# Boese0601/RC-MVSNet

Measured on AMD Instinct MI355X. Metric: ref-scenes/sec (DTU 3-view 512x640, D=48/32/8), higher is better.
Workload: dtype f32; 1 GPU; BASELINE configs[1]: CascadeMVSNet_eval.forward, DTU-shaped 3 views 512x640, D=(48,32,8), batch 1 per GPU, fp32, random-init seeded weights; views=3, height=512, width=640, parallelism=scene-per-gpu x1, ranks=1, procs_per_gpu=1, rccl_ranks=0

## Files before the change

rc_mvsnet_amd/casmvsnet.py:

```python
import os

FP16_PAIR_DEFAULT = True
ONE_BY_ONE_MFMA = os.environ.get("RCMVS_1X1_MFMA", "1") != "0"
HEAD_PAIR = os.environ.get("RCMVS_HEAD_PAIR", "1") != "0"
CONV11_PROB = int(os.environ.get("RCMVS_CONV11_PROB", "1"))
CONV_TILE = os.environ.get("RCMVS_CONV_TILE", "1") != "0"
CONV_STEM = os.environ.get("RCMVS_CONV_STEM", "1") != "0"
CONV_PAIR = os.environ.get("RCMVS_CONV_PAIR", "1") != "0"
DEEP_PAIR = os.environ.get("RCMVS_DEEP_PAIR", "1") != "0"

import torch
import torch.nn as nn
import torch.nn.functional as F

from . import ops
from ._lib import RcmvsError


def _nhwc(x):
    x = x.contiguous().float()
    return ops.rgb_to_nhwc4(x) if x.shape[1] == 3 else ops.to_channels_last(x)


def _param(mod, name):
    p = mod._parameters.get(name)
    return p if p is not None else getattr(mod, name)


def _packed_of(module, make):
    w = module.conv.weight
    key = (w.data_ptr(), w._version, str(w.device))
    c = module.__dict__.get("_rcmvs_pack")
    if c is None or c[0] != key:
        c = module.__dict__["_rcmvs_pack"] = (key, make(w.detach()))
    return c[1]


def _affine_of(m):
    if getattr(m, "gn", None) is not None:
        raise RcmvsError(f"{type(m).__name__}: GroupNorm blocks are not provided (the reference builds every block with norm='batch_norm')")
    if m.bn is not None:
        return _bn_fold(m.bn)
    b = m.conv.bias
    if b is None:
        return None, None
    return torch.ones_like(b, dtype=torch.float32), b.detach().float().contiguous()


def _same2(v, n):
    return tuple(v) == (n, n)


def _conv2d_block_cl(m, t):
    conv = m.conv
    K = conv.kernel_size[0]
    st = conv.stride[0]
    if (not _same2(conv.kernel_size, K) or K not in (1, 3, 5) or not _same2(conv.padding, K // 2) or not _same2(conv.stride, st)
            or st not in (1, 2) or not _same2(conv.dilation, 1) or conv.groups != 1 or conv.padding_mode != "zeros"):
# ... 618 lines not shown
        depth = None
        bounds = None
        need_fill = False
        pair = getattr(self, "fp16_pair", None)
        if pair is None:
            pair = FP16_PAIR_DEFAULT if os.environ.get("RCMVS_FP16_PAIR") is None else os.environ["RCMVS_FP16_PAIR"] == "1"
        if pair and B == 1:
            bounds = getattr(self, "_pair_bounds", None)
            if getattr(self, "_is_replica", False):
                bounds = torch.zeros(self.num_stage, CostRegNet.BOUND_ROWS, ops.ABSMAX_FLOATS, device=imgs.device, dtype=torch.float32)
            elif bounds is None or bounds.device != imgs.device:
                bounds = self._pair_bounds = torch.zeros(self.num_stage, CostRegNet.BOUND_ROWS, ops.ABSMAX_FLOATS, device=imgs.device, dtype=torch.float32)
            else:
                need_fill = True
        if homographies is None:
            if self.num_stage <= 4:
                rots, transs = ops.compose_homography_stages([proj_matrices["stage{}".format(k + 1)].contiguous().float() for k in range(self.num_stage)],
                                                             zero=bounds if need_fill else None)
                need_fill = False
            else:
                rt = [ops.compose_homography(proj_matrices["stage{}".format(k + 1)].contiguous().float()) for k in range(self.num_stage)]
                rots, transs = [r for r, _ in rt], [t for _, t in rt]
        if need_fill:
            bounds.zero_()
        for s in range(self.num_stage):
            key = "stage{}".format(s + 1)
            scale = int(self.stage_infos[key]["scale"])
            D = self.ndepths[s]
            bound_kept = False
            if feats_cl is not None:
                fk, bound_kept = feats_cl[key](bounds[s][0] if bounds is not None else None)
                h, w, C = fk.shape[1:]
                f_cl = fk.view(B, V, h, w, C)
            else:
                C, h, w = features[key].shape[1:]
                f_cl = ops.to_channels_last(features[key].contiguous()).view(B, V, h, w, C)
            if homographies is not None:
                rot, trans = homographies[key]
            else:
                rot, trans = rots[s], transs[s]
            planes = ops.hypothesis_planes(depth, depth_values, (H, W), scale, D, self.depth_interals_ratio[s])
            var = ops.warp_variance(f_cl, rot, trans, planes, D, uniform_planes=depth is None)
            cr = self._cr(s)
            vmax = None
            if bounds is not None:
                vmax = bounds[s]
                if not bound_kept:
                    ops.absmax(f_cl, square=True, out=vmax[0])
            plan = cr.hip_plan()
            if vmax is not None and HEAD_PAIR and (CONV11_PROB == 2 or (CONV11_PROB == 1 and D == 8)):
                depth, conf = cr.features_cl(var, vmax, plan, logits=True, planes=planes)
            else:
                x8 = cr.features_cl(var, vmax, plan)
                depth, conf = ops.depth_head(x8, plan["prob"], planes, x_absmax=vmax[CostRegNet.BOUND_ROWS - 1] if vmax is not None and HEAD_PAIR else None)
            out = {"depth": depth, "photometric_confidence": conf}
            if self.TRAIN_VARIANT:
                small_cl = ops.resize_rgb_cl(imgs.reshape(B * V, 3, H, W).contiguous(), (h, w)).view(B, V, h, w, 3)
                out["volume_feature_no_ref"] = ops.warp_noref(f_cl, small_cl, rot, trans, planes, D, square_first=True)
            outputs[key] = out
            outputs.update(out)
        return outputs

    def _forward_train_hip(self, imgs, proj_matrices, depth_values):
        from . import train_ops
        B, V, _, H, W = imgs.shape
        imgs = imgs.float()
        depth_values = depth_values.contiguous().float()
        fv = self.feature.forward_train_cl(imgs.transpose(0, 1).reshape(V * B, 3, H, W), segments=V)
        features = [{k: f[v * B:(v + 1) * B] for k, f in fv.items()} for v in range(V)]
        outputs = {}
        depth = None
        for s in range(self.num_stage):
            key = "stage{}".format(s + 1)
            scale = int(self.stage_infos[key]["scale"])
            D = self.ndepths[s]
            f_cl = torch.stack([f[key] for f in features], dim=1).contiguous()
            h, w = f_cl.shape[2:4]
            with torch.no_grad():
                rot, trans = ops.compose_homography(proj_matrices[key].contiguous().float())
                prev = depth.detach() if depth is not None else None
                planes = ops.hypothesis_planes(prev, depth_values, (H, W), scale, D, self.depth_interals_ratio[s])
                small_cl = None
                if self.TRAIN_VARIANT:
                    small_cl = ops.resize_rgb_cl(imgs.reshape(B * V, 3, H, W).contiguous(), (h, w)).view(B, V, h, w, 3)
            res = ops.WarpVarianceFn.apply(f_cl, rot, trans, planes, D, small_cl)
            var, noref = res if self.TRAIN_VARIANT else (res, None)
            cr = self._cr(s)
            x8 = cr.features_cl_train(var)
            prev_live = depth
            depth, conf = train_ops.ProbDepthHeadFn.apply(x8, cr.prob.weight, planes)
            if prev_live is not None and self.grad_method != "detach":
                up = F.interpolate(prev_live.unsqueeze(1), [H, W], mode="bilinear", align_corners=False)
                base = F.interpolate(up, [h, w], mode="bilinear", align_corners=False).squeeze(1)
                depth = depth + (base - base.detach())
            out = {"depth": depth, "photometric_confidence": conf}
            if self.TRAIN_VARIANT:
                out["volume_feature_no_ref"] = noref
            outputs[key] = out
            outputs.update(out)
        return outputs

    def _run(self, imgs, proj_matrices, depth_values):
        if _hip_inference(self, imgs, depth_values):
            return self._forward_hip(imgs, proj_matrices, depth_values)
        if _hip_training(self, imgs, depth_values):
            return self._forward_train_hip(imgs, proj_matrices, depth_values)
        _unsupported(self, imgs, depth_values)
# ... 16 lines not shown
```

rc_mvsnet_amd/csrc/depth_head.hip:

```cpp
#include "common.h"

namespace rcmvs {

int conv3d_lds_launch(const float* x, const float* wp, const float* scale, const float* shift, const float* res, float* y,
                      int B, int D, int H, int W, int Ci, int Co, int relu, hipStream_t st, int lds_cfg);
bool prob_head_fused_supported(int D, int H, int W);
bool prob_pair_supported(int D, int H, int W);
int prob_pair_launch(const float* x, const float* wimg, const float* xmax, float* y, const float* planes, float* depth, float* conf,
                     int B, int D, int H, int W, bool fuse, int zc_force, hipStream_t st);
long long prob_pair_blob_offset();
int prob_head_fused_launch(const float* x, const float* wp, const float* planes, float* depth, float* conf, float* prob,
                           int B, int D, int H, int W, hipStream_t st);

template <int LP, bool KEEP = true>
__global__ __launch_bounds__(256) void softmax_regress_kernel(float* __restrict__ prob, const float* __restrict__ planes,
                                                               float* __restrict__ depth, float* __restrict__ conf, int D, long long hw) {
    constexpr int MAXK = 16;
    const int b = blockIdx.y;
    const int j = threadIdx.x % LP;
    const long long p = ((long long)blockIdx.x * blockDim.x + threadIdx.x) / LP;
    const bool live = p < hw;
    float* col = prob + (long long)b * D * hw + (live ? p : 0);
    float v[MAXK];
    float mx = -INFINITY;
#pragma unroll
    for (int i = 0; i < MAXK; ++i) {
        const int k = j + i * LP;
        v[i] = (k < D) ? col[(long long)k * hw] : -INFINITY;
        mx = fmaxf(mx, v[i]);
    }
#pragma unroll
    for (int m = 1; m < LP; m <<= 1) mx = fmaxf(mx, __shfl_xor(mx, m));
    float sum = 0.0f;
#pragma unroll
    for (int i = 0; i < MAXK; ++i) {
        v[i] = (j + i * LP < D) ? expf(v[i] - mx) : 0.0f;
        sum += v[i];
    }
#pragma unroll
    for (int m = 1; m < LP; m <<= 1) sum += __shfl_xor(sum, m);
    const float2 pl = reinterpret_cast<const float2*>(planes)[(long long)b * hw + (live ? p : 0)];
    float dsum = 0.0f, isum = 0.0f;
#pragma unroll
    for (int i = 0; i < MAXK; ++i) {
        const int k = j + i * LP;
        v[i] = v[i] / sum;
        if (k < D) {
            if (KEEP && live) col[(long long)k * hw] = v[i];
            dsum = fmaf(v[i], fmaf((float)k, pl.y, pl.x), dsum);
            isum = fmaf(v[i], (float)k, isum);
        }
    }
#pragma unroll
    for (int m = 1; m < LP; m <<= 1) { dsum += __shfl_xor(dsum, m); isum += __shfl_xor(isum, m); }
    int idx = (int)isum;
    idx = idx < 0 ? 0 : (idx > D - 1 ? D - 1 : idx);
    float c = 0.0f;
#pragma unroll
    for (int i = 0; i < MAXK; ++i) {
        const int k = j + i * LP;
        if (k < D && k >= idx - 1 && k <= idx + 2) c += v[i];
    }
#pragma unroll
    for (int m = 1; m < LP; m <<= 1) c += __shfl_xor(c, m);
    if (live && j == 0) {
        depth[(long long)b * hw + p] = dsum;
        conf[(long long)b * hw + p] = c;
    }
}

}

using namespace rcmvs;

static int depth_head_fwd(const float* x, const float* xmax, const float* w_prob, const float* planes, float* depth, float* conf, float* prob,
                          int B, int D, int h, int w, int impl, void* stream) {
    RCMVS_REQUIRE(x && w_prob && planes && depth && conf, "depth_head_fwd: null pointer");
    RCMVS_REQUIRE(B > 0 && D > 0 && h > 0 && w > 0, "depth_head_fwd: bad sizes");
    RCMVS_REQUIRE(D <= 64, "depth_head_fwd: at most 64 depth hypotheses per stage (got %d)", D);
    hipStream_t st = as_stream(stream);
    const int zc_force = (impl >> 8) & 0xff;
    const bool pair = xmax && !(impl & 4) && prob_pair_supported(D, h, w);
    int rc;
    if (pair && D == 8 && !(impl & 1))
        return prob_pair_launch(x, w_prob + prob_pair_blob_offset(), xmax, prob, planes, depth, conf, B, D, h, w, true, 0, st);
    if (!pair && !(impl & 1) && prob_head_fused_supported(D, h, w)) return prob_head_fused_launch(x, w_prob, planes, depth, conf, prob, B, D, h, w, st);
    RCMVS_REQUIRE(prob, "depth_head_fwd: prob is required for D = %d (it doubles as the logit scratch; only the D = 8 form runs without)", D);
    if (pair) rc = prob_pair_launch(x, w_prob + prob_pair_blob_offset(), xmax, prob, nullptr, nullptr, nullptr, B, D, h, w, false, zc_force, st);
    else rc = conv3d_lds_launch(x, w_prob, nullptr, nullptr, nullptr, prob, B, D, h, w, 8, 1, 0, st, ((impl & 2) ? 16 : 0) | (zc_force << 8));
    if (rc) return rc;
    const long long hw = (long long)h * w;
    const bool keep = !(impl & 8);
#define RCMVS_SOFTMAX(LP) do { if (keep) hipLaunchKernelGGL((softmax_regress_kernel<LP, true>), dim3((unsigned)cdiv(hw * LP, 256), B), dim3(256), 0, st, prob, planes, depth, conf, D, hw); \
                               else hipLaunchKernelGGL((softmax_regress_kernel<LP, false>), dim3((unsigned)cdiv(hw * LP, 256), B), dim3(256), 0, st, prob, planes, depth, conf, D, hw); } while (0)
    if (D <= 16) RCMVS_SOFTMAX(1);
    else if (D <= 32) RCMVS_SOFTMAX(2);
    else RCMVS_SOFTMAX(4);
#undef RCMVS_SOFTMAX
    return launch_status("depth_head_fwd");
}

extern "C" int rcmvs_softmax_head_fwd(float* prob, const float* planes, float* depth, float* conf, int B, int D, int h, int w, int keep, void* stream) {
    RCMVS_REQUIRE(prob && planes && depth && conf, "softmax_head_fwd: null pointer");
    RCMVS_REQUIRE(B > 0 && D > 0 && h > 0 && w > 0, "softmax_head_fwd: bad sizes");
    RCMVS_REQUIRE(D <= 64, "softmax_head_fwd: at most 64 depth hypotheses per stage (got %d)", D);
    hipStream_t st = as_stream(stream);
    const long long hw = (long long)h * w;
#define RCMVS_SOFTMAX(LP) do { if (keep) hipLaunchKernelGGL((softmax_regress_kernel<LP, true>), dim3((unsigned)cdiv(hw * LP, 256), B), dim3(256), 0, st, prob, planes, depth, conf, D, hw); \
                               else hipLaunchKernelGGL((softmax_regress_kernel<LP, false>), dim3((unsigned)cdiv(hw * LP, 256), B), dim3(256), 0, st, prob, planes, depth, conf, D, hw); } while (0)
    if (D <= 16) RCMVS_SOFTMAX(1);
    else if (D <= 32) RCMVS_SOFTMAX(2);
    else RCMVS_SOFTMAX(4);
#undef RCMVS_SOFTMAX
    return launch_status("softmax_head_fwd");
}

extern "C" int rcmvs_depth_head_fwd(const float* x, const float* w_prob, const float* planes, float* depth, float* conf, float* prob,
                                    int B, int D, int h, int w, void* stream) {
    return depth_head_fwd(x, nullptr, w_prob, planes, depth, conf, prob, B, D, h, w, 0, stream);
}
extern "C" int rcmvs_depth_head_scaled_fwd(const float* x, const float* x_absmax, const float* w_prob, const float* planes, float* depth, float* conf,
                                           float* prob, int B, int D, int h, int w, int impl, void* stream) {
    return depth_head_fwd(x, x_absmax, w_prob, planes, depth, conf, prob, B, D, h, w, impl, stream);
}
```

rc_mvsnet_amd/csrc/prob_pair.hip:

```cpp
#include "common.h"
#include "x3_pieces.h"
#include <type_traits>

namespace rcmvs {

constexpr int PP_TH = 8, PP_TW = 32, PP_HH = PP_TH + 2, PP_HW = PP_TW + 2;
constexpr int PP_PIECE = PP_HH * PP_HW * 16;
constexpr int PP_BUF = 2 * PP_PIECE;
constexpr int PP_NLD = (PP_HH * PP_HW * 2 + 255) / 256;
constexpr int PP_NJ = 3, PP_STEP = 14;

long long prob_pair_weight_floats() { return 4 + 3 * 2 * 64 * 4; }

__global__ void prob_pair_pack_kernel(const float* __restrict__ w, unsigned short* __restrict__ img, const float* __restrict__ wsc) {
    const int t = blockIdx.x * blockDim.x + threadIdx.x;
    if (t >= 3 * 64 * 8) return;
    const int c = t & 7, lane = (t >> 3) & 63, r = t >> 9;
    const int m = lane & 15, kh = lane >> 4, g = m >> 2, kw = m & 3;
    float v = 0.0f;
    if (g < 3 && kw < 3 && kh < 3) {
        const int kd = (g + r) % 3;
        v = w[c * 27 + (kd * 3 + kh) * 3 + kw];
    }
    const float sw = wsc[0];
    if (t == 0) { float* hdr = reinterpret_cast<float*>(img); hdr[0] = sw; hdr[1] = wsc[1]; hdr[2] = 0.0f; hdr[3] = 0.0f; }
    const float vs = v * sw;
    const _Float16 h = (_Float16)vs;
    const _Float16 l = (_Float16)(vs - (float)h);
    const int base = 8 + ((r * 2) * 64 + lane) * 8 + c;
    img[base] = __builtin_bit_cast(unsigned short, h);
    img[base + 64 * 8] = __builtin_bit_cast(unsigned short, l);
}

int prob_pair_pack(const float* w, float* img, const float* wsc, hipStream_t st) {
    hipLaunchKernelGGL(prob_pair_pack_kernel, dim3(6), dim3(256), 0, st, w, reinterpret_cast<unsigned short*>(img), wsc);
    return launch_status("prob_pair_pack");
}

template <int FUSE_D>
__global__ __launch_bounds__(256, 4) void prob_pair_kernel(
    const float* __restrict__ x, const x3_u32x4* __restrict__ wimg, const float* __restrict__ xmax, float* __restrict__ y,
    int D, int H, int W, int tiles_w, int tiles_h, int zchunk,
    const float* __restrict__ planes, float* __restrict__ depth, float* __restrict__ conf) {
    constexpr int LGB = FUSE_D > 0 ? FUSE_D * 256 * 4 : 0;
    __shared__ __attribute__((aligned(16))) x3_byte smem[2 * PP_BUF + LGB + 16];
    constexpr int OOB = 0x7ffffff0;
    const int tid = threadIdx.x, lane = tid & 63;
    const int wave = __builtin_amdgcn_readfirstlane(tid >> 6);
    const int n = lane & 15, kq = lane >> 4;
    const int b = blockIdx.z, zc = blockIdx.y;
    const unsigned t2 = xcd_remap(blockIdx.x, gridDim.x);
    const int tw = t2 % tiles_w, th = t2 / tiles_w;
    const int h0 = th * PP_TH, w0 = tw * PP_TW, z0 = zc * zchunk;
    const int z1 = min(D, z0 + zchunk);
    const int nplanes = z1 - z0 + 2;
    const int plane_bytes = H * W * 32;
    const float xmax_lane = xmax[lane * 16];
    const float whdr = reinterpret_cast<const float*>(wimg)[1];
    __amdgpu_buffer_rsrc_t xrs = __builtin_amdgcn_make_buffer_rsrc(const_cast<float*>(x + (long long)b * D * H * W * 8), (short)0, D * plane_bytes, 0x00020000);
    __amdgpu_buffer_rsrc_t yrs = __builtin_amdgcn_make_buffer_rsrc(y ? y + (long long)b * D * H * W : nullptr, (short)0, y ? D * H * W * 4 : 0, 0x00020000);
    int goff[PP_NLD], ls[PP_NLD];
#pragma unroll
    for (int i = 0; i < PP_NLD; ++i) {
        const int e = tid + i * 256;
        const int v = e >> 1, c4 = e & 1;
        const int hh = v / PP_HW, hw_ = v - hh * PP_HW;
        const int ih = h0 + hh - 1, iw = w0 + hw_ - 1;
        const bool has = e < PP_HH * PP_HW * 2;
        goff[i] = (has && ih >= 0 && ih < H && iw >= 0 && iw < W) ? ((ih * W + iw) * 8 + c4 * 4) * 4 : OOB;
        ls[i] = has ? v * 16 + c4 * 8 : -1;
    }
    x3_u32x4 pf[PP_NLD];
    auto fetch = [&](int z) {
        const bool zin = z >= 0 && z < D;
        const int zoff = zin ? z * plane_bytes : 0;
#pragma unroll
        for (int i = 0; i < PP_NLD; ++i) pf[i] = __builtin_amdgcn_raw_buffer_load_b128(xrs, zin ? goff[i] : OOB, zoff, 0);
    };
    x3_u32x4 A[3][2];
#pragma unroll
    for (int r = 0; r < 3; ++r)
#pragma unroll
        for (int p = 0; p < 2; ++p) A[r][p] = wimg[1 + (r * 2 + p) * 64 + lane];
    fetch(z0 - 1);
    float bound = xmax_lane;
#pragma unroll
    for (int m = 32; m > 0; m >>= 1) bound = fmaxf(bound, __shfl_xor(bound, m));
    float xinv;
    const float xs_scale = x3_pow2_scale(bound, xinv);
    const float unscale = xinv * whdr;
    auto stash = [&](int buf) {
#pragma unroll
        for (int i = 0; i < PP_NLD; ++i) {
            x3_u32x2 h, l;
            x3_split4h(__builtin_bit_cast(x3_f32x4, pf[i]) * xs_scale, h, l);
            if (ls[i] >= 0) {
                *reinterpret_cast<x3_u32x2*>(smem + buf * PP_BUF + ls[i]) = h;
                *reinterpret_cast<x3_u32x2*>(smem + buf * PP_BUF + PP_PIECE + ls[i]) = l;
            }
        }
    };
    stash(0);
    fetch(z0);
    __syncthreads();
    int baddr[2][PP_NJ], ooff[2][PP_NJ];
#pragma unroll
    for (int rr = 0; rr < 2; ++rr)
#pragma unroll
        for (int j = 0; j < PP_NJ; ++j) {
            const int row = 2 * wave + rr, q = min(PP_STEP * j + n, PP_HW - 1);
            baddr[rr][j] = ((row + (kq < 3 ? kq : 0)) * PP_HW + q) * 16;
            const int wl = PP_STEP * j + n, oh = h0 + row, ow = w0 + wl;
            const bool ok = n < PP_STEP && wl < PP_TW && oh < H && ow < W;
            ooff[rr][j] = FUSE_D > 0 ? (ok ? (row * PP_TW + wl) * 4 : -1) : (ok ? (oh * W + ow) * 4 : OOB);
        }
    x3_f32x4 acc[2][PP_NJ];
#pragma unroll
    for (int rr = 0; rr < 2; ++rr)
#pragma unroll
        for (int j = 0; j < PP_NJ; ++j) acc[rr][j] = (x3_f32x4){0.f, 0.f, 0.f, 0.f};
    float* const lg = reinterpret_cast<float*>(smem + 2 * PP_BUF);

    auto body = [&](auto rtag, int i, int buf) {
        constexpr int R = decltype(rtag)::value, G = (2 - R + 3) % 3;
        const x3_byte* pb = smem + buf * PP_BUF;
#pragma unroll
        for (int j = 0; j < PP_NJ; ++j) {
            x3_u32x4 bh[2], bl[2];
#pragma unroll
            for (int rr = 0; rr < 2; ++rr) {
                bh[rr] = *reinterpret_cast<const x3_u32x4*>(pb + baddr[rr][j]);
                bl[rr] = *reinterpret_cast<const x3_u32x4*>(pb + PP_PIECE + baddr[rr][j]);
            }
#pragma unroll
            for (int rr = 0; rr < 2; ++rr) acc[rr][j] = x3_mfma<2>(A[R][0], bh[rr], acc[rr][j]);
#pragma unroll
            for (int rr = 0; rr < 2; ++rr) acc[rr][j] = x3_mfma<2>(A[R][0], bl[rr], acc[rr][j]);
#pragma unroll
            for (int rr = 0; rr < 2; ++rr) acc[rr][j] = x3_mfma<2>(A[R][1], bh[rr], acc[rr][j]);
        }
        const int o = i - 2;
        const bool mine = kq == G;
#pragma unroll
        for (int rr = 0; rr < 2; ++rr)
#pragma unroll
            for (int j = 0; j < PP_NJ; ++j) {
                x3_f32x4& a = acc[rr][j];
                const float a0 = a[0], a1 = a[1], a2 = a[2];
                const float s1 = __builtin_bit_cast(float, __builtin_amdgcn_update_dpp(0, __builtin_bit_cast(int, a1), 0x101, 0xf, 0xf, true));
                const float s2 = __builtin_bit_cast(float, __builtin_amdgcn_update_dpp(0, __builtin_bit_cast(int, a2), 0x102, 0xf, 0xf, true));
                const float v = ((a0 + s1) + s2) * unscale;
                if (o >= 0 && o < z1 - z0) {
                    if constexpr (FUSE_D > 0) {
                        if (mine && ooff[rr][j] >= 0) lg[o * 256 + ooff[rr][j] / 4] = v;
                    } else {
                        __builtin_amdgcn_raw_buffer_store_b32(__float_as_uint(v), yrs, mine ? ooff[rr][j] : OOB, (z0 + o) * H * W * 4, 0);
                    }
                }
                a[0] = mine ? 0.0f : a[0]; a[1] = mine ? 0.0f : a[1]; a[2] = mine ? 0.0f : a[2];
            }
        if (i + 1 < nplanes) {
            stash(buf ^ 1);
            if (i + 2 < nplanes) fetch(z0 - 1 + i + 2);
        }
        __syncthreads();
    };
    using R0 = std::integral_constant<int, 0>;
    using R1 = std::integral_constant<int, 1>;
    using R2 = std::integral_constant<int, 2>;
    for (int i = 0; i < nplanes; i += 3) {
        body(R0{}, i, i & 1);
        if (i + 1 < nplanes) body(R1{}, i + 1, (i + 1) & 1);
        if (i + 2 < nplanes) body(R2{}, i + 2, i & 1);
    }
    if constexpr (FUSE_D > 0) {
        const int lw = tid % PP_TW, lh = tid / PP_TW;
        const int oh = h0 + lh, ow = w0 + lw;
        const bool live = oh < H && ow < W;
        const int ooffp = live ? (oh * W + ow) * 4 : OOB;
        float v[FUSE_D];
        float mx = -INFINITY;
#pragma unroll
        for (int k = 0; k < FUSE_D; ++k) { v[k] = lg[k * 256 + tid]; mx = fmaxf(mx, v[k]); }
        float sum = 0.0f;
#pragma unroll
        for (int k = 0; k < FUSE_D; ++k) { v[k] = expf(v[k] - mx); sum += v[k]; }
        const long long hw = (long long)H * W;
        const long long pix = live ? (long long)oh * W + ow : 0;
        const float2 pl = reinterpret_cast<const float2*>(planes)[(long long)b * hw + pix];
        float dsum = 0.0f, isum = 0.0f;
#pragma unroll
        for (int k = 0; k < FUSE_D; ++k) {
            v[k] = v[k] / sum;
            if (y) __builtin_amdgcn_raw_buffer_store_b32(__float_as_uint(v[k]), yrs, ooffp, k * H * W * 4, 0);
            dsum = fmaf(v[k], fmaf((float)k, pl.y, pl.x), dsum);
            isum = fmaf(v[k], (float)k, isum);
        }
        int idx = (int)isum;
        idx = idx < 0 ? 0 : (idx > FUSE_D - 1 ? FUSE_D - 1 : idx);
        float c = 0.0f;
#pragma unroll
        for (int k = 0; k < FUSE_D; ++k)
            if (k >= idx - 1 && k <= idx + 2) c += v[k];
        if (live) {
            depth[(long long)b * hw + pix] = dsum;
            conf[(long long)b * hw + pix] = c;
        }
    }
}

static int prob_pair_zchunk(int tiles, int D) {
    static int slots = 0;
    if (!slots) {
        hipDeviceProp_t prop;
        int dev = 0;
        slots = (hipGetDevice(&dev) == hipSuccess && hipGetDeviceProperties(&prop, dev) == hipSuccess && prop.multiProcessorCount > 0 ? prop.multiProcessorCount : 256) * 5;
    }
    long long best = -1; int zc = D < 8 ? D : 8;
    for (int c = D < 16 ? D : 16; c >= 2; --c) {
        const long long blocks = (long long)tiles * ((D + c - 1) / c);
        const long long cost = ((blocks + slots - 1) / slots) * (c + 2);
        if (best < 0 || cost < best) { best = cost; zc = c; }
    }
    return zc;
}

bool prob_pair_supported(int D, int H, int W) { return D > 0 && (long long)D * H * W * 32 < 0x7ffffff0LL; }

int prob_pair_launch(const float* x, const float* wimg, const float* xmax, float* y, const float* planes, float* depth, float* conf,
                     int B, int D, int H, int W, bool fuse, int zc_force, hipStream_t st) {
    if (!prob_pair_supported(D, H, W)) return fail(-1, "prob_pair: volume too large for 32-bit offsets");
    const int tw_ = (W + PP_TW - 1) / PP_TW, th_ = (H + PP_TH - 1) / PP_TH;
    if (fuse) {
        if (D != 8) return fail(-1, "prob_pair: the one-launch head needs D = 8 (got %d)", D);
        hipLaunchKernelGGL(prob_pair_kernel<8>, dim3(tw_ * th_, 1, B), dim3(256), 0, st, x, reinterpret_cast<const x3_u32x4*>(wimg), xmax, y, D, H, W, tw_, th_, D,
                           planes, depth, conf);
        return launch_status("depth_head(pair, fused)");
    }
    const int zc = zc_force ? (zc_force < D ? zc_force : D) : prob_pair_zchunk(B * tw_ * th_, D);
    hipLaunchKernelGGL(prob_pair_kernel<0>, dim3(tw_ * th_, (D + zc - 1) / zc, B), dim3(256), 0, st, x, reinterpret_cast<const x3_u32x4*>(wimg), xmax, y, D, H, W, tw_, th_, zc,
                       (const float*)nullptr, (float*)nullptr, (float*)nullptr);
    return launch_status("prob_pair");
}

}
```

rc_mvsnet_amd/ops.py:

```python
import ctypes
import os

import torch

from . import _lib

K1_EVENTS = None
K1_UNIFORM_PLANES = _lib.CONSTANTS["RCMVS_K1_UNIFORM_PLANES"]
K1_FAST_BLEND = _lib.CONSTANTS["RCMVS_K1_FAST_BLEND"]
CONV_EVENTS = None


_FIRST_STREAM = {}


def _multi_stream_allowed():
    return os.environ.get("GPU_MAX_HW_QUEUES") == "1" or os.environ.get("RCMVS_ALLOW_MULTI_STREAM") == "1"


def _stream():
    st = torch.cuda.current_stream()
    key = st.device_index
    first = _FIRST_STREAM.setdefault(key, st.cuda_stream)
    if first != st.cuda_stream and not _multi_stream_allowed():
# ... 408 lines not shown
    y = torch.empty((N, H, W, CO), device=lat.device, dtype=torch.float32)
    _lib.call("rcmvs_fpn_out_fused", _chk(lat, "lat"), _chk(up, "up"), _chk(w_inner_packed.blob, "w_inner"), _chk(b_inner, "b_inner"),
              _chk(w_out_packed.blob, "w_out"), _chk(y, "y"), N, H, W, CL, CM, CO, _stream())
    return y


FPN_FOLDED_FLOATS = _lib.CONSTANTS["RCMVS_FPN_FOLDED_FLOATS"]


def pack_fpn_folded(w_inner, b_inner, w_out):
    wi = w_inner.detach().double().reshape(32, 8)
    wo = w_out.detach().double()
    b = b_inner.detach().double()
    wb = torch.einsum("mi,omyx->yxio", wi, wo)
    bt = torch.einsum("m,omyx->yxo", b, wo)
    inside = {0: (1, 2), 1: (0, 1, 2), 2: (0, 1)}
    bs = torch.stack([torch.stack([sum(bt[ky, kx] for ky in inside[cy] for kx in inside[cx]) for cx in range(3)]) for cy in range(3)])
    rows = lambda p: ((0,), (1, 2)) if p == 0 else ((0, 1), (2,))
    wa = torch.zeros(2, 2, 2, 2, 32, 8, dtype=torch.float64, device=wo.device)
    for py in range(2):
        for px in range(2):
            for ry in range(2):
                for rx in range(2):
                    for ky in rows(py)[ry]:
                        for kx in rows(px)[rx]:
                            wa[py, px, ry, rx] += wo[:, :, ky, kx].t()
    tab = torch.cat((wb.reshape(-1), bs.reshape(-1), wa.reshape(-1))).float().contiguous()
    assert tab.numel() == FPN_FOLDED_FLOATS
    return tab


def pack_fpn_folded_mfma(tables):
    if tables.numel() != FPN_FOLDED_FLOATS:
        raise _lib.RcmvsError("pack_fpn_folded_mfma: expects the tables of pack_fpn_folded")
    img = torch.empty((_lib.load().rcmvs_fpn_folded_mfma_floats(),), device=tables.device, dtype=torch.float32)
    _lib.call("rcmvs_fpn_folded_mfma_pack", _chk(tables, "tables"), _chk(img, "image"), _stream())
    return img


def fpn_out_folded(lat, up, tables, ysq_absmax=None):
    N, H, W, CL = lat.shape
    mfma = tables.numel() == _lib.load().rcmvs_fpn_folded_mfma_floats()
    if CL != 8 or tuple(up.shape) != (N, H // 2, W // 2, 32) or not (mfma or tables.numel() == FPN_FOLDED_FLOATS):
        raise _lib.RcmvsError(f"fpn_out_folded: lat {tuple(lat.shape)} / up {tuple(up.shape)} / {tables.numel()} table floats do not fit 8 -> 32 -> 8")
    y = torch.empty((N, H, W, 8), device=lat.device, dtype=torch.float32)
    _lib.call("rcmvs_fpn_out_folded_mfma" if mfma else "rcmvs_fpn_out_folded", _chk(lat, "lat"), _chk(up, "up"), _chk(tables, "tables"), _chk(y, "y"),
              _opt(ysq_absmax, "ysq_absmax"), N, H, W, _stream())
    return y


DEPTH_HEAD_IMPL = 0


def depth_head(x8, w_prob_packed, planes, want_prob=False, x_absmax=None):
    B, D, h, w, C = x8.shape
    if C != 8:
        raise _lib.RcmvsError("depth_head: the prob conv takes 8 channels")
    if x_absmax is not None and w_prob_packed.images != IMG_ALL:
        raise _lib.RcmvsError("depth_head: the fp16-pair form reads an image that a selectively packed weight does not hold")
    depth = torch.empty((B, h, w), device=x8.device, dtype=torch.float32)
    conf = torch.empty((B, h, w), device=x8.device, dtype=torch.float32)
    one_launch = D == 8 and not (DEPTH_HEAD_IMPL & 1)
    prob = None if one_launch and not want_prob else torch.empty((B, D, h, w), device=x8.device, dtype=torch.float32)
    _lib.call("rcmvs_depth_head_scaled_fwd", _chk(x8, "x8"), _opt(x_absmax, "x_absmax"), _chk(w_prob_packed.blob, "w_prob"), _chk(planes, "planes"),
              _chk(depth, "depth"), _chk(conf, "conf"), _opt(prob, "prob"), B, D, h, w,
              DEPTH_HEAD_IMPL | (0 if want_prob else 8), _stream())
    return (depth, conf, prob) if want_prob else (depth, conf)


def conv11_prob(t, t_absmax, w11_packed, scale, shift, res, res_absmax, coef, w_prob_packed, zchunk=0, planes=None):
    B, Dt, Ht, Wt, C = t.shape
    if C != 16 or tuple(res.shape) != (B, 2 * Dt, 2 * Ht, 2 * Wt, 8):
        raise _lib.RcmvsError(f"conv11_prob: t {tuple(t.shape)} / res {tuple(res.shape)} are not (B,Dt,Ht,Wt,16) / (B,2Dt,2Ht,2Wt,8)")
    if w11_packed.images != IMG_ALL or w_prob_packed.images != IMG_ALL:
        raise _lib.RcmvsError("conv11_prob: needs the full weight blobs (a selectively packed weight does not hold the fp16-pair images)")
    fused = planes is not None and Dt == 4
    logits = depth = conf = None
    if fused:
        depth = torch.empty((B, 2 * Ht, 2 * Wt), device=t.device, dtype=torch.float32)
        conf = torch.empty((B, 2 * Ht, 2 * Wt), device=t.device, dtype=torch.float32)
    else:
        logits = torch.empty((B, 2 * Dt, 2 * Ht, 2 * Wt), device=t.device, dtype=torch.float32)
    _lib.call("rcmvs_conv11_prob_fwd", _chk(t, "t"), _chk(t_absmax, "t_absmax"), _chk(w11_packed.blob, "w11"), _chk(scale, "scale"),
              _chk(shift, "shift"), _chk(res, "res"), _chk(res_absmax, "res_absmax"), _chk(coef, "coef"),
              _chk(w_prob_packed.blob, "w_prob"), _opt(logits, "logits"), _opt(planes if fused else None, "planes"),
              _opt(depth, "depth"), _opt(conf, "conf"), B, Dt, Ht, Wt, int(zchunk), _stream())
    if fused:
        return depth, conf
    if planes is not None:
        return softmax_head(logits, planes)
    return logits


def softmax_head(logits, planes, keep_prob=False):
    B, D, h, w = logits.shape
    depth = torch.empty((B, h, w), device=logits.device, dtype=torch.float32)
    conf = torch.empty((B, h, w), device=logits.device, dtype=torch.float32)
    _lib.call("rcmvs_softmax_head_fwd", _chk(logits, "logits"), _chk(planes, "planes"), _chk(depth, "depth"), _chk(conf, "conf"),
              B, D, h, w, int(bool(keep_prob)), _stream())
    return depth, conf


def resize_planes(x, out_planes, pad_channels_to=None):
    B, C, D, h, w = x.shape
    Cp = C if pad_channels_to is None else pad_channels_to
    y = torch.empty((B, out_planes, h, w, Cp), device=x.device, dtype=torch.float32)
    _lib.call("rcmvs_resize_planes_fwd", _chk(x, "x"), _chk(y, "y"), B, C, Cp, D, out_planes, h, w, _stream())
    return y


def gu_sample(pseudo_depth, img0, pix, eps, u, cam):
    H, W = pseudo_depth.shape
    N, S = eps.shape
    dev = eps.device
    f = lambda *shape: torch.empty(shape, device=dev, dtype=torch.float32)
    z, pts, ndc, dirs, rdepth, target = f(N, S), f(N, S, 3), f(N, S, 3), f(N, 3), f(N), f(N, 3)
    _lib.call("rcmvs_gu_sample_fwd", _chk(pseudo_depth, "pseudo_depth"), _chk(img0, "img0"), _chk(pix, "pix", torch.int32),
              _chk(eps, "eps"), _chk(u, "u"), _chk(cam, "cam"), _chk(z, "z"), _chk(pts, "pts"),
              _chk(ndc, "ndc"), _chk(dirs, "dirs"), _chk(rdepth, "rays_depth"), _chk(target, "target"),
# ... 66 lines not shown
```

Before: 946.1 ref-scenes/s.

## Fuse prob conv and softmax regression into one launch for D=48/32 stages

Extends the fp16-pair prob conv kernel with a one-launch head variant for any D up to 64. Each tile keeps all logit planes in dynamic LDS and runs the softmax/depth regression in-kernel, so the logit volume no longer goes to global memory and the separate softmax kernel is dropped. It uses a smaller 4-row tile by default and deeper z-prefetch (three slots), raises the dynamic LDS limit, and factors the softmax column into a shared header. The large per-block LDS footprint (for D=48) limits occupancy, and the shorter tiles mean more halo reloads.

```diff
diff --git a/rc_mvsnet_amd/casmvsnet.py b/rc_mvsnet_amd/casmvsnet.py
--- a/rc_mvsnet_amd/casmvsnet.py
+++ b/rc_mvsnet_amd/casmvsnet.py
@@ -4,6 +4,7 @@
 ONE_BY_ONE_MFMA = os.environ.get("RCMVS_1X1_MFMA", "1") != "0"
 HEAD_PAIR = os.environ.get("RCMVS_HEAD_PAIR", "1") != "0"
 CONV11_PROB = int(os.environ.get("RCMVS_CONV11_PROB", "1"))
+HEAD_ONE_LAUNCH = os.environ.get("RCMVS_HEAD_ONE_LAUNCH", "1") != "0"
 CONV_TILE = os.environ.get("RCMVS_CONV_TILE", "1") != "0"
 CONV_STEM = os.environ.get("RCMVS_CONV_STEM", "1") != "0"
 CONV_PAIR = os.environ.get("RCMVS_CONV_PAIR", "1") != "0"
@@ -728,7 +729,8 @@
                 depth, conf = cr.features_cl(var, vmax, plan, logits=True, planes=planes)
             else:
                 x8 = cr.features_cl(var, vmax, plan)
-                depth, conf = ops.depth_head(x8, plan["prob"], planes, x_absmax=vmax[CostRegNet.BOUND_ROWS - 1] if vmax is not None and HEAD_PAIR else None)
+                depth, conf = ops.depth_head(x8, plan["prob"], planes, x_absmax=vmax[CostRegNet.BOUND_ROWS - 1] if vmax is not None and HEAD_PAIR else None,
+                                             one_launch=HEAD_ONE_LAUNCH)
             out = {"depth": depth, "photometric_confidence": conf}
             if self.TRAIN_VARIANT:
                 small_cl = ops.resize_rgb_cl(imgs.reshape(B * V, 3, H, W).contiguous(), (h, w)).view(B, V, h, w, 3)
diff --git a/rc_mvsnet_amd/csrc/depth_head.hip b/rc_mvsnet_amd/csrc/depth_head.hip
--- a/rc_mvsnet_amd/csrc/depth_head.hip
+++ b/rc_mvsnet_amd/csrc/depth_head.hip
@@ -1,4 +1,5 @@
 #include "common.h"
+#include "softmax_head.h"
 
 namespace rcmvs {
 
@@ -15,54 +16,14 @@
 template <int LP, bool KEEP = true>
 __global__ __launch_bounds__(256) void softmax_regress_kernel(float* __restrict__ prob, const float* __restrict__ planes,
                                                                float* __restrict__ depth, float* __restrict__ conf, int D, long long hw) {
-    constexpr int MAXK = 16;
     const int b = blockIdx.y;
     const int j = threadIdx.x % LP;
     const long long p = ((long long)blockIdx.x * blockDim.x + threadIdx.x) / LP;
     const bool live = p < hw;
     float* col = prob + (long long)b * D * hw + (live ? p : 0);
-    float v[MAXK];
-    float mx = -INFINITY;
-#pragma unroll
-    for (int i = 0; i < MAXK; ++i) {
-        const int k = j + i * LP;
-        v[i] = (k < D) ? col[(long long)k * hw] : -INFINITY;
-        mx = fmaxf(mx, v[i]);
-    }
-#pragma unroll
-    for (int m = 1; m < LP; m <<= 1) mx = fmaxf(mx, __shfl_xor(mx, m));
-    float sum = 0.0f;
-#pragma unroll
-    for (int i = 0; i < MAXK; ++i) {
-        v[i] = (j + i * LP < D) ? expf(v[i] - mx) : 0.0f;
-        sum += v[i];
-    }
-#pragma unroll
-    for (int m = 1; m < LP; m <<= 1) sum += __shfl_xor(sum, m);
     const float2 pl = reinterpret_cast<const float2*>(planes)[(long long)b * hw + (live ? p : 0)];
-    float dsum = 0.0f, isum = 0.0f;
-#pragma unroll
-    for (int i = 0; i < MAXK; ++i) {
-        const int k = j + i * LP;
-        v[i] = v[i] / sum;
-        if (k < D) {
-            if (KEEP && live) col[(long long)k * hw] = v[i];
-            dsum = fmaf(v[i], fmaf((float)k, pl.y, pl.x), dsum);
-            isum = fmaf(v[i], (float)k, isum);
-        }
-    }
-#pragma unroll
-    for (int m = 1; m < LP; m <<= 1) { dsum += __shfl_xor(dsum, m); isum += __shfl_xor(isum, m); }
-    int idx = (int)isum;
-    idx = idx < 0 ? 0 : (idx > D - 1 ? D - 1 : idx);
-    float c = 0.0f;
-#pragma unroll
-    for (int i = 0; i < MAXK; ++i) {
-        const int k = j + i * LP;
-        if (k < D && k >= idx - 1 && k <= idx + 2) c += v[i];
-    }
-#pragma unroll
-    for (int m = 1; m < LP; m <<= 1) c += __shfl_xor(c, m);
+    float dsum, c;
+    softmax_head_column<LP, KEEP>(col, hw, D, j, live, pl, dsum, c);
     if (live && j == 0) {
         depth[(long long)b * hw + p] = dsum;
         conf[(long long)b * hw + p] = c;
@@ -84,8 +45,10 @@
     int rc;
     if (pair && D == 8 && !(impl & 1))
         return prob_pair_launch(x, w_prob + prob_pair_blob_offset(), xmax, prob, planes, depth, conf, B, D, h, w, true, 0, st);
+    if (pair && D != 8 && (impl & 8) && !(impl & 16))
+        return prob_pair_launch(x, w_prob + prob_pair_blob_offset(), xmax, nullptr, planes, depth, conf, B, D, h, w, true, 0, st);
     if (!pair && !(impl & 1) && prob_head_fused_supported(D, h, w)) return prob_head_fused_launch(x, w_prob, planes, depth, conf, prob, B, D, h, w, st);
-    RCMVS_REQUIRE(prob, "depth_head_fwd: prob is required for D = %d (it doubles as the logit scratch; only the D = 8 form runs without)", D);
+    RCMVS_REQUIRE(prob, "depth_head_fwd: prob is required for D = %d (it doubles as the logit scratch; only the one-launch forms run without)", D);
     if (pair) rc = prob_pair_launch(x, w_prob + prob_pair_blob_offset(), xmax, prob, nullptr, nullptr, nullptr, B, D, h, w, false, zc_force, st);
     else rc = conv3d_lds_launch(x, w_prob, nullptr, nullptr, nullptr, prob, B, D, h, w, 8, 1, 0, st, ((impl & 2) ? 16 : 0) | (zc_force << 8));
     if (rc) return rc;
diff --git a/rc_mvsnet_amd/csrc/prob_pair.hip b/rc_mvsnet_amd/csrc/prob_pair.hip
--- a/rc_mvsnet_amd/csrc/prob_pair.hip
+++ b/rc_mvsnet_amd/csrc/prob_pair.hip
@@ -1,14 +1,22 @@
 #include "common.h"
+#include "softmax_head.h"
 #include "x3_pieces.h"
+#include <atomic>
+#include <cstdlib>
 #include <type_traits>
 
 namespace rcmvs {
 
-constexpr int PP_TH = 8, PP_TW = 32, PP_HH = PP_TH + 2, PP_HW = PP_TW + 2;
-constexpr int PP_PIECE = PP_HH * PP_HW * 16;
-constexpr int PP_BUF = 2 * PP_PIECE;
-constexpr int PP_NLD = (PP_HH * PP_HW * 2 + 255) / 256;
+constexpr int PP_TW = 32, PP_HW = PP_TW + 2;
 constexpr int PP_NJ = 3, PP_STEP = 14;
+template <int RR>
+struct PPTile {
+    static constexpr int TH = 4 * RR, HH = TH + 2, PIX = TH * PP_TW;
+    static constexpr int PIECE = HH * PP_HW * 16;
+    static constexpr int BUF = 2 * PIECE;
+    static constexpr int NLD = (HH * PP_HW * 2 + 255) / 256;
+};
+__host__ __device__ inline int prob_pair_logit_stride(int pix, int D) { const int lp = softmax_head_lanes(D); return pix + (lp > 1 ? 64 / lp : 0); }
 
 long long prob_pair_weight_floats() { return 4 + 3 * 2 * 64 * 4; }
 
@@ -37,13 +45,17 @@
     return launch_status("prob_pair_pack");
 }
 
-template <int FUSE_D>
-__global__ __launch_bounds__(256, 4) void prob_pair_kernel(
+template <int FUSE_D, int RR = 2>
+__global__ __launch_bounds__(256, (FUSE_D < 0 && RR == 2) ? 2 : 4) void prob_pair_kernel(
     const float* __restrict__ x, const x3_u32x4* __restrict__ wimg, const float* __restrict__ xmax, float* __restrict__ y,
     int D, int H, int W, int tiles_w, int tiles_h, int zchunk,
     const float* __restrict__ planes, float* __restrict__ depth, float* __restrict__ conf) {
-    constexpr int LGB = FUSE_D > 0 ? FUSE_D * 256 * 4 : 0;
+    using T = PPTile<RR>;
+    constexpr int PP_TH = T::TH, PP_HH = T::HH, PP_PIECE = T::PIECE, PP_BUF = T::BUF, PP_NLD = T::NLD;
+    constexpr int LGB = FUSE_D > 0 ? FUSE_D * T::PIX * 4 : 0;
+    constexpr int PFD = FUSE_D < 0 ? 3 : 1;
     __shared__ __attribute__((aligned(16))) x3_byte smem[2 * PP_BUF + LGB + 16];
+    extern __shared__ __attribute__((aligned(16))) x3_byte dyn_lg[];
     constexpr int OOB = 0x7ffffff0;
     const int tid = threadIdx.x, lane = tid & 63;
     const int wave = __builtin_amdgcn_readfirstlane(tid >> 6);
@@ -70,79 +82,104 @@
         goff[i] = (has && ih >= 0 && ih < H && iw >= 0 && iw < W) ? ((ih * W + iw) * 8 + c4 * 4) * 4 : OOB;
         ls[i] = has ? v * 16 + c4 * 8 : -1;
     }
-    x3_u32x4 pf[PP_NLD];
-    auto fetch = [&](int z) {
+    x3_u32x4 pf[PFD][PP_NLD];
+    auto fetch = [&](auto slot, int z) {
         const bool zin = z >= 0 && z < D;
         const int zoff = zin ? z * plane_bytes : 0;
 #pragma unroll
-        for (int i = 0; i < PP_NLD; ++i) pf[i] = __builtin_amdgcn_raw_buffer_load_b128(xrs, zin ? goff[i] : OOB, zoff, 0);
+        for (int i = 0; i < PP_NLD; ++i) pf[decltype(slot)::value][i] = __builtin_amdgcn_raw_buffer_load_b128(xrs, zin ? goff[i] : OOB, zoff, 0);
     };
+    using S0 = std::integral_constant<int, 0>;
+    using S1 = std::integral_constant<int, (PFD > 1 ? 1 : 0)>;
+    using S2 = std::integral_constant<int, (PFD > 1 ? 2 : 0)>;
     x3_u32x4 A[3][2];
 #pragma unroll
     for (int r = 0; r < 3; ++r)
 #pragma unroll
         for (int p = 0; p < 2; ++p) A[r][p] = wimg[1 + (r * 2 + p) * 64 + lane];
-    fetch(z0 - 1);
+    fetch(S0{}, z0 - 1);
     float bound = xmax_lane;
 #pragma unroll
     for (int m = 32; m > 0; m >>= 1) bound = fmaxf(bound, __shfl_xor(bound, m));
     float xinv;
     const float xs_scale = x3_pow2_scale(bound, xinv);
     const float unscale = xinv * whdr;
-    auto stash = [&](int buf) {
+    auto stash = [&](auto slot, int buf) {
 #pragma unroll
         for (int i = 0; i < PP_NLD; ++i) {
             x3_u32x2 h, l;
-            x3_split4h(__builtin_bit_cast(x3_f32x4, pf[i]) * xs_scale, h, l);
+            x3_split4h(__builtin_bit_cast(x3_f32x4, pf[decltype(slot)::value][i]) * xs_scale, h, l);
             if (ls[i] >= 0) {
                 *reinterpret_cast<x3_u32x2*>(smem + buf * PP_BUF + ls[i]) = h;
                 *reinterpret_cast<x3_u32x2*>(smem + buf * PP_BUF + PP_PIECE + ls[i]) = l;
             }
         }
     };
-    stash(0);
-    fetch(z0);
+    stash(S0{}, 0);
+    if constexpr (PFD == 3) {
+        fetch(S1{}, z0);
+        fetch(S2{}, z0 + 1);
+        fetch(S0{}, z0 + 2);
+    } else {
+        fetch(S0{}, z0);
+    }
     __syncthreads();
-    int baddr[2][PP_NJ], ooff[2][PP_NJ];
-#pragma unroll
-    for (int rr = 0; rr < 2; ++rr)
+    const int lgs = FUSE_D > 0 ? T::PIX : prob_pair_logit_stride(T::PIX, D);
+    int baddr[RR][PP_NJ], ooff[RR][PP_NJ];
+#pragma unroll
+    for (int rr = 0; rr < RR; ++rr)
 #pragma unroll
         for (int j = 0; j < PP_NJ; ++j) {
-            const int row = 2 * wave + rr, q = min(PP_STEP * j + n, PP_HW - 1);
+            const int row = RR * wave + rr, q = min(PP_STEP * j + n, PP_HW - 1);
             baddr[rr][j] = ((row + (kq < 3 ? kq : 0)) * PP_HW + q) * 16;
             const int wl = PP_STEP * j + n, oh = h0 + row, ow = w0 + wl;
             const bool ok = n < PP_STEP && wl < PP_TW && oh < H && ow < W;
-            ooff[rr][j] = FUSE_D > 0 ? (ok ? (row * PP_TW + wl) * 4 : -1) : (ok ? (oh * W + ow) * 4 : OOB);
-        }
-    x3_f32x4 acc[2][PP_NJ];
-#pragma unroll
-    for (int rr = 0; rr < 2; ++rr)
+            ooff[rr][j] = FUSE_D != 0 ? (ok ? (row * PP_TW + wl) * 4 : -1) : (ok ? (oh * W + ow) * 4 : OOB);
+        }
+    x3_f32x4 acc[RR][PP_NJ];
+#pragma unroll
+    for (int rr = 0; rr < RR; ++rr)
 #pragma unroll
         for (int j = 0; j < PP_NJ; ++j) acc[rr][j] = (x3_f32x4){0.f, 0.f, 0.f, 0.f};
-    float* const lg = reinterpret_cast<float*>(smem + 2 * PP_BUF);
+    float* const lg = reinterpret_cast<float*>(FUSE_D < 0 ? dyn_lg : smem + 2 * PP_BUF);
 
     auto body = [&](auto rtag, int i, int buf) {
         constexpr int R = decltype(rtag)::value, G = (2 - R + 3) % 3;
         const x3_byte* pb = smem + buf * PP_BUF;
-#pragma unroll
-        for (int j = 0; j < PP_NJ; ++j) {
-            x3_u32x4 bh[2], bl[2];
-#pragma unroll
-            for (int rr = 0; rr < 2; ++rr) {
-                bh[rr] = *reinterpret_cast<const x3_u32x4*>(pb + baddr[rr][j]);
-                bl[rr] = *reinterpret_cast<const x3_u32x4*>(pb + PP_PIECE + baddr[rr][j]);
-            }
-#pragma unroll
-            for (int rr = 0; rr < 2; ++rr) acc[rr][j] = x3_mfma<2>(A[R][0], bh[rr], acc[rr][j]);
-#pragma unroll
-            for (int rr = 0; rr < 2; ++rr) acc[rr][j] = x3_mfma<2>(A[R][0], bl[rr], acc[rr][j]);
-#pragma unroll
-            for (int rr = 0; rr < 2; ++rr) acc[rr][j] = x3_mfma<2>(A[R][1], bh[rr], acc[rr][j]);
+        if constexpr (RR == 1) {
+            x3_u32x4 bh[PP_NJ], bl[PP_NJ];
+#pragma unroll
+            for (int j = 0; j < PP_NJ; ++j) {
+                bh[j] = *reinterpret_cast<const x3_u32x4*>(pb + baddr[0][j]);
+                bl[j] = *reinterpret_cast<const x3_u32x4*>(pb + PP_PIECE + baddr[0][j]);
+            }
+#pragma unroll
+            for (int j = 0; j < PP_NJ; ++j) acc[0][j] = x3_mfma<2>(A[R][0], bh[j], acc[0][j]);
+#pragma unroll
+            for (int j = 0; j < PP_NJ; ++j) acc[0][j] = x3_mfma<2>(A[R][0], bl[j], acc[0][j]);
+#pragma unroll
+            for (int j = 0; j < PP_NJ; ++j) acc[0][j] = x3_mfma<2>(A[R][1], bh[j], acc[0][j]);
+        } else {
+#pragma unroll
+            for (int j = 0; j < PP_NJ; ++j) {
+                x3_u32x4 bh[RR], bl[RR];
+#pragma unroll
+                for (int rr = 0; rr < RR; ++rr) {
+                    bh[rr] = *reinterpret_cast<const x3_u32x4*>(pb + baddr[rr][j]);
+                    bl[rr] = *reinterpret_cast<const x3_u32x4*>(pb + PP_PIECE + baddr[rr][j]);
+                }
+#pragma unroll
+                for (int rr = 0; rr < RR; ++rr) acc[rr][j] = x3_mfma<2>(A[R][0], bh[rr], acc[rr][j]);
+#pragma unroll
+                for (int rr = 0; rr < RR; ++rr) acc[rr][j] = x3_mfma<2>(A[R][0], bl[rr], acc[rr][j]);
+#pragma unroll
+                for (int rr = 0; rr < RR; ++rr) acc[rr][j] = x3_mfma<2>(A[R][1], bh[rr], acc[rr][j]);
+            }
         }
         const int o = i - 2;
         const bool mine = kq == G;
 #pragma unroll
-        for (int rr = 0; rr < 2; ++rr)
+        for (int rr = 0; rr < RR; ++rr)
 #pragma unroll
             for (int j = 0; j < PP_NJ; ++j) {
                 x3_f32x4& a = acc[rr][j];
@@ -151,8 +188,8 @@
                 const float s2 = __builtin_bit_cast(float, __builtin_amdgcn_update_dpp(0, __builtin_bit_cast(int, a2), 0x102, 0xf, 0xf, true));
                 const float v = ((a0 + s1) + s2) * unscale;
                 if (o >= 0 && o < z1 - z0) {
-                    if constexpr (FUSE_D > 0) {
-                        if (mine && ooff[rr][j] >= 0) lg[o * 256 + ooff[rr][j] / 4] = v;
+                    if constexpr (FUSE_D != 0) {
+                        if (mine && ooff[rr][j] >= 0) lg[o * lgs + ooff[rr][j] / 4] = v;
                     } else {
                         __builtin_amdgcn_raw_buffer_store_b32(__float_as_uint(v), yrs, mine ? ooff[rr][j] : OOB, (z0 + o) * H * W * 4, 0);
                     }
@@ -160,8 +197,9 @@
                 a[0] = mine ? 0.0f : a[0]; a[1] = mine ? 0.0f : a[1]; a[2] = mine ? 0.0f : a[2];
             }
         if (i + 1 < nplanes) {
-            stash(buf ^ 1);
-            if (i + 2 < nplanes) fetch(z0 - 1 + i + 2);
+            using SN = std::integral_constant<int, PFD == 3 ? (R + 1) % 3 : 0>;
+            stash(SN{}, buf ^ 1);
+            if (i + 1 + PFD < nplanes) fetch(SN{}, z0 - 1 + i + 1 + PFD);
         }
         __syncthreads();
     };
@@ -173,6 +211,29 @@
         if (i + 1 < nplanes) body(R1{}, i + 1, (i + 1) & 1);
         if (i + 2 < nplanes) body(R2{}, i + 2, i & 1);
     }
+    if constexpr (FUSE_D < 0) {
+        auto head = [&](auto lptag) {
+            constexpr int LP = decltype(lptag)::value;
+            const long long hw = (long long)H * W;
+            const int j = tid % LP;
+            for (int p0 = 0; p0 < T::PIX; p0 += 256 / LP) {
+                const int lp_ = p0 + tid / LP;
+                const int oh = h0 + lp_ / PP_TW, ow = w0 + lp_ % PP_TW;
+                const bool live = lp_ < T::PIX && oh < H && ow < W;
+                const long long pix = live ? (long long)oh * W + ow : 0;
+                const float2 pl = reinterpret_cast<const float2*>(planes)[(long long)b * hw + pix];
+                float dsum, c;
+                softmax_head_column<LP, false>(const_cast<const float*>(lg) + (live ? lp_ : 0), lgs, D, j, live, pl, dsum, c);
+                if (live && j == 0) {
+                    depth[(long long)b * hw + pix] = dsum;
+                    conf[(long long)b * hw + pix] = c;
+                }
+            }
+        };
+        if (D <= 16) head(std::integral_constant<int, 1>{});
+        else if (D <= 32) head(std::integral_constant<int, 2>{});
+        else head(std::integral_constant<int, 4>{});
+    }
     if constexpr (FUSE_D > 0) {
         const int lw = tid % PP_TW, lh = tid / PP_TW;
         const int oh = h0 + lh, ow = w0 + lw;
@@ -227,15 +288,41 @@
 
 bool prob_pair_supported(int D, int H, int W) { return D > 0 && (long long)D * H * W * 32 < 0x7ffffff0LL; }
 
+template <int RR>
+static int prob_pair_head_launch(const float* x, const float* wimg, const float* xmax, const float* planes, float* depth, float* conf,
+                                 int B, int D, int H, int W, hipStream_t st) {
+    using T = PPTile<RR>;
+    constexpr int LDS_MAX = 160 * 1024 - (2 * T::BUF + 16);
+    const int lds = D * prob_pair_logit_stride(T::PIX, D) * 4;
+    if (lds > LDS_MAX) return fail(-1, "prob_pair: %d logit planes of a %d-row tile do not fit the LDS", D, T::TH);
+    static std::atomic<bool> raised[64];
+    int dev = 0;
+    if (hipGetDevice(&dev) != hipSuccess || dev < 0 || dev >= 64) return fail(-1, "prob_pair: cannot query the device");
+    if (!raised[dev].load(std::memory_order_acquire)) {
+        if (hipFuncSetAttribute((const void*)prob_pair_kernel<-1, RR>, hipFuncAttributeMaxDynamicSharedMemorySize, LDS_MAX) != hipSuccess)
+            return fail(-1, "prob_pair: cannot raise the dynamic LDS limit to %d bytes", LDS_MAX);
+        raised[dev].store(true, std::memory_order_release);
+    }
+    const int tw_ = (W + PP_TW - 1) / PP_TW, th_ = (H + T::TH - 1) / T::TH;
+    hipLaunchKernelGGL((prob_pair_kernel<-1, RR>), dim3(tw_ * th_, 1, B), dim3(256), lds, st, x, reinterpret_cast<const x3_u32x4*>(wimg), xmax, (float*)nullptr,
+                       D, H, W, tw_, th_, D, planes, depth, conf);
+    return launch_status("depth_head(pair, one launch)");
+}
+
 int prob_pair_launch(const float* x, const float* wimg, const float* xmax, float* y, const float* planes, float* depth, float* conf,
                      int B, int D, int H, int W, bool fuse, int zc_force, hipStream_t st) {
     if (!prob_pair_supported(D, H, W)) return fail(-1, "prob_pair: volume too large for 32-bit offsets");
-    const int tw_ = (W + PP_TW - 1) / PP_TW, th_ = (H + PP_TH - 1) / PP_TH;
-    if (fuse) {
-        if (D != 8) return fail(-1, "prob_pair: the one-launch head needs D = 8 (got %d)", D);
+    const int tw_ = (W + PP_TW - 1) / PP_TW, th_ = (H + PPTile<2>::TH - 1) / PPTile<2>::TH;
+    if (fuse && D == 8) {
         hipLaunchKernelGGL(prob_pair_kernel<8>, dim3(tw_ * th_, 1, B), dim3(256), 0, st, x, reinterpret_cast<const x3_u32x4*>(wimg), xmax, y, D, H, W, tw_, th_, D,
                            planes, depth, conf);
         return launch_status("depth_head(pair, fused)");
+    }
+    if (fuse) {
+        if (D > 64) return fail(-1, "prob_pair: the one-launch head takes at most 64 planes (got %d)", D);
+        const char* t = getenv("RCMVS_PP_TILE");
+        if (t && t[0] == '2') return prob_pair_head_launch<2>(x, wimg, xmax, planes, depth, conf, B, D, H, W, st);
+        return prob_pair_head_launch<1>(x, wimg, xmax, planes, depth, conf, B, D, H, W, st);
     }
     const int zc = zc_force ? (zc_force < D ? zc_force : D) : prob_pair_zchunk(B * tw_ * th_, D);
     hipLaunchKernelGGL(prob_pair_kernel<0>, dim3(tw_ * th_, (D + zc - 1) / zc, B), dim3(256), 0, st, x, reinterpret_cast<const x3_u32x4*>(wimg), xmax, y, D, H, W, tw_, th_, zc,
diff --git a/rc_mvsnet_amd/csrc/softmax_head.h b/rc_mvsnet_amd/csrc/softmax_head.h
--- /dev/null
+++ b/rc_mvsnet_amd/csrc/softmax_head.h
@@ -0,0 +1,56 @@
+#pragma once
+#include "common.h"
+
+namespace rcmvs {
+
+__host__ __device__ inline int softmax_head_lanes(int D) { return D <= 16 ? 1 : (D <= 32 ? 2 : 4); }
+
+template <int LP, bool KEEP, typename T, typename S>
+__device__ __forceinline__ void softmax_head_column(T* __restrict__ col, S stride, int D, int j, bool live, float2 pl, float& depth, float& conf) {
+    constexpr int MAXK = 16;
+    float v[MAXK];
+    float mx = -INFINITY;
+#pragma unroll
+    for (int i = 0; i < MAXK; ++i) {
+        const int k = j + i * LP;
+        v[i] = (k < D) ? col[(S)k * stride] : -INFINITY;
+        mx = fmaxf(mx, v[i]);
+    }
+#pragma unroll
+    for (int m = 1; m < LP; m <<= 1) mx = fmaxf(mx, __shfl_xor(mx, m));
+    float sum = 0.0f;
+#pragma unroll
+    for (int i = 0; i < MAXK; ++i) {
+        v[i] = (j + i * LP < D) ? expf(v[i] - mx) : 0.0f;
+        sum += v[i];
+    }
+#pragma unroll
+    for (int m = 1; m < LP; m <<= 1) sum += __shfl_xor(sum, m);
+    float dsum = 0.0f, isum = 0.0f;
+#pragma unroll
+    for (int i = 0; i < MAXK; ++i) {
+        const int k = j + i * LP;
+        v[i] = v[i] / sum;
+        if (k < D) {
+            if constexpr (KEEP) { if (live) col[(S)k * stride] = v[i]; }
+            dsum = fmaf(v[i], fmaf((float)k, pl.y, pl.x), dsum);
+            isum = fmaf(v[i], (float)k, isum);
+        }
+    }
+#pragma unroll
+    for (int m = 1; m < LP; m <<= 1) { dsum += __shfl_xor(dsum, m); isum += __shfl_xor(isum, m); }
+    int idx = (int)isum;
+    idx = idx < 0 ? 0 : (idx > D - 1 ? D - 1 : idx);
+    float c = 0.0f;
+#pragma unroll
+    for (int i = 0; i < MAXK; ++i) {
+        const int k = j + i * LP;
+        if (k < D && k >= idx - 1 && k <= idx + 2) c += v[i];
+    }
+#pragma unroll
+    for (int m = 1; m < LP; m <<= 1) c += __shfl_xor(c, m);
+    depth = dsum;
+    conf = c;
+}
+
+}
diff --git a/rc_mvsnet_amd/ops.py b/rc_mvsnet_amd/ops.py
--- a/rc_mvsnet_amd/ops.py
+++ b/rc_mvsnet_amd/ops.py
@@ -484,7 +484,7 @@
 DEPTH_HEAD_IMPL = 0
 
 
-def depth_head(x8, w_prob_packed, planes, want_prob=False, x_absmax=None):
+def depth_head(x8, w_prob_packed, planes, want_prob=False, x_absmax=None, one_launch=True):
     B, D, h, w, C = x8.shape
     if C != 8:
         raise _lib.RcmvsError("depth_head: the prob conv takes 8 channels")
@@ -492,11 +492,14 @@
         raise _lib.RcmvsError("depth_head: the fp16-pair form reads an image that a selectively packed weight does not hold")
     depth = torch.empty((B, h, w), device=x8.device, dtype=torch.float32)
     conf = torch.empty((B, h, w), device=x8.device, dtype=torch.float32)
-    one_launch = D == 8 and not (DEPTH_HEAD_IMPL & 1)
-    prob = None if one_launch and not want_prob else torch.empty((B, D, h, w), device=x8.device, dtype=torch.float32)
+    impl = DEPTH_HEAD_IMPL | (0 if want_prob else 8) | (0 if one_launch else 16)
+    if D == 8:
+        scratch = bool(impl & 1)
+    else:
+        scratch = want_prob or x_absmax is None or bool(impl & (4 | 16)) or D * h * w * 32 >= 0x7ffffff0
+    prob = torch.empty((B, D, h, w), device=x8.device, dtype=torch.float32) if want_prob or scratch else None
     _lib.call("rcmvs_depth_head_scaled_fwd", _chk(x8, "x8"), _opt(x_absmax, "x_absmax"), _chk(w_prob_packed.blob, "w_prob"), _chk(planes, "planes"),
-              _chk(depth, "depth"), _chk(conf, "conf"), _opt(prob, "prob"), B, D, h, w,
-              DEPTH_HEAD_IMPL | (0 if want_prob else 8), _stream())
+              _chk(depth, "depth"), _chk(conf, "conf"), _opt(prob, "prob"), B, D, h, w, impl, _stream())
     return (depth, conf, prob) if want_prob else (depth, conf)
 
 
```

After: 936.6 ref-scenes/s. 0.99x the previous value.
